# getreu/stringsext

Measured on AMD Instinct MI355X. Metric: GiB/s scanned, higher is better.
Workload: dtype u8

## Files before the change

stringsext_amd/csrc/sx_ctx.hpp:

```cpp
#pragma once
#include <hip/hip_runtime_api.h>
#include <stdio.h>
#include <stdlib.h>
#include <string.h>
#include <errno.h>
#include <fcntl.h>
#include <sys/mman.h>
#include <sys/stat.h>
#include <unistd.h>

#include <algorithm>
#include <atomic>
#include <chrono>
#include <condition_variable>
#include <deque>
#include <functional>
#include <mutex>
#include <string>
#include <thread>
#include <unordered_map>
#include <vector>

#include "sx_host.hpp"
#include "sx_switches.hpp"
// ... 81 lines not shown
    uint64_t* h_tot = nullptr;
    const uint32_t* grid_of_scan = nullptr; uint32_t grid_sub = 0; const uint8_t* grid_data = nullptr; uint64_t grid_len = 0;
    uint8_t* h_small = nullptr;
    std::vector<hipEvent_t> wave_ev;
};


}

struct sx_result {
    sx::Result r;
};

struct sx_ctx {
    std::shared_ptr<sx::PinnedPool> pool = std::make_shared<sx::PinnedPool>();
    std::shared_ptr<std::atomic<uint64_t>> dev_epoch = std::make_shared<std::atomic<uint64_t>>(0);
    std::vector<sx::Mission> missions;
    std::vector<sx::ScannerState> states;
    std::vector<sx::MissionDev> dev;
    bool host_only = false;
    bool sharded_call = false, single_piece = true;
    int device = -1;
    sx_options opt{};
    sx::Switches sw;
    std::string err;
    sx_stats stats{};
    hipStream_t scan_stream = nullptr, post_stream = nullptr;
    uint8_t* d_cache = nullptr;
    uint64_t d_cache_cap = 0;
    hipStream_t merge_copy_stream = nullptr;
    hipEvent_t merge_ev[3] = { nullptr, nullptr, nullptr };
    uint8_t* d_merge = nullptr; uint64_t d_merge_cap = 0, merge_out_room = 0, merge_n_out = 0;
    uint8_t* d_result = nullptr; uint64_t d_result_cap = 0;
    uint8_t* d_result_up = nullptr; uint64_t d_result_up_cap = 0;
    bool merge_async = false;
    bool merge_copy_pending[2] = { false, false };
    uint64_t merge_parts = 0;
    uint64_t merged_out_bytes = 0;
    double out_density = 0;
    hipEvent_t ev_interleaved = nullptr;
    std::atomic<bool> interleave_pending{ false };
    std::mutex mu;
    std::mutex err_mu;
    std::recursive_mutex grow_mu;
    void set_err(std::string text) { std::lock_guard<std::mutex> g(err_mu); err = std::move(text); }
    unsigned n_cus = 256, scan_blocks_per_cu = 8;
    hipStream_t copy_stream = nullptr;
    hipStream_t d2h_stream = nullptr;
    uint8_t* ing_pin[2] = { nullptr, nullptr };
    uint8_t* ing_dev[2] = { nullptr, nullptr };
    uint64_t ing_cap = 0, ing_dev_cap = 0;
    uint32_t region_cap = 64;
    std::vector<uint32_t> dense;
    uint8_t* d_input = nullptr;
    uint64_t d_input_cap = 0;
    uint64_t ondemand_fetches = 0;
    std::vector<uint64_t> last_runs;
    std::vector<char> wave_pred;
    std::vector<double> wave_density;
    std::vector<char> wave_off;
    std::vector<sx::RunList> shard_runs;
    bool shard_runs_valid = false;
    uint64_t shard_runs_off = 0, shard_runs_len = 0;
    const void* shard_runs_ptr = nullptr;
    uint8_t* h_pin = nullptr;   uint64_t h_pin_cap = 0;
    uint8_t* h_pin2 = nullptr;  uint64_t h_pin2_cap = 0;
    uint8_t* d_scratch = nullptr; uint64_t d_scratch_cap = 0;
};

#define HIP_TRY(ctx, expr)                                                                     \
    do {                                                                                       \
        hipError_t e_ = (expr);                                                                \
        if (e_ != hipSuccess) {                                                                \
            (ctx)->set_err(std::string(#expr) + ": " + hipGetErrorString(e_));                 \
            return SX_E_HIP;                                                                   \
        }                                                                                      \
    } while (0)

namespace sx {

class SparseDeviceBytes : public ByteView {
public:
    SparseDeviceBytes(sx_ctx* ctx, const uint8_t* d_base, uint64_t len = 0) : ctx_(ctx), d_base_(d_base), len_(len) {}
    void add(uint64_t lo, uint64_t hi, const uint8_t* p) { segs_.push_back({ lo, hi, p }); }
    void add_copy(uint64_t lo, uint64_t hi, const uint8_t* p) {
        owned_.emplace_back(p, p + (hi - lo));
        segs_.push_back({ lo, hi, owned_.back().data() });
    }
    bool empty() const { return segs_.empty(); }
    const uint8_t* span(uint64_t off, size_t n, size_t* hint) override {
        size_t a = *hint < segs_.size() ? *hint : 0;
        if (!(a < segs_.size() && segs_[a].lo <= off)) a = 0;
        size_t steps = 0;
        while (a < segs_.size() && segs_[a].hi <= off && steps < 8) { a++; steps++; }
        if (!(a < segs_.size() && segs_[a].lo <= off && off < segs_[a].hi)) {
            size_t lo = 0, hi = segs_.size();
            while (lo < hi) {
                size_t mid = (lo + hi) / 2;
                if (segs_[mid].hi <= off) lo = mid + 1; else hi = mid;
            }
            a = lo;
        }
        if (a < segs_.size() && segs_[a].lo <= off && off + n <= segs_[a].hi) { *hint = a; return segs_[a].p + (off - segs_[a].lo); }
        std::lock_guard<std::mutex> g(mu_);
        if (len_) {
            const uint64_t b = off / kBlock;
            if (off + n <= std::min<uint64_t>(len_, (b + 1) * kBlock)) {
                auto it = blocks_.find(b);
                if (it == blocks_.end()) {
                    const uint64_t lo = b * kBlock, hi = std::min<uint64_t>(len_, lo + kBlock);
                    std::vector<uint8_t> v((size_t)(hi - lo));
                    if (hipMemcpy(v.data(), d_base_ + lo, (size_t)(hi - lo), hipMemcpyDeviceToHost) != hipSuccess) memset(v.data(), 0, v.size());
                    ctx_->ondemand_fetches++;
                    it = blocks_.emplace(b, std::move(v)).first;
                }
                return it->second.data() + (off - b * kBlock);
            }
        }
        extra_.emplace_back(n);
        if (hipMemcpy(extra_.back().data(), d_base_ + off, n, hipMemcpyDeviceToHost) != hipSuccess)
            memset(extra_.back().data(), 0, n);
        ctx_->ondemand_fetches++;
        return extra_.back().data();
    }

private:
    struct Seg { uint64_t lo, hi; const uint8_t* p; };
    sx_ctx* ctx_;
    const uint8_t* d_base_;
    uint64_t len_ = 0;
    static constexpr uint64_t kBlock = 65536;
    std::unordered_map<uint64_t, std::vector<uint8_t>> blocks_;
    std::vector<Seg> segs_;
    std::deque<std::vector<uint8_t>> extra_, owned_;
    std::mutex mu_;
};

int ensure_pinned(sx_ctx* ctx, uint64_t bytes);
int ensure_pinned2(sx_ctx* ctx, uint64_t bytes);
int read_back_sync(sx_ctx* ctx, sx::MissionDev& d, hipStream_t s, void* host_dst, const void* dev_src, size_t bytes);
int read_back_async(sx_ctx* ctx, hipStream_t s, void* pinned_dst, const void* dev_src, size_t bytes);
int ensure_scratch(sx_ctx* ctx, uint64_t bytes);
int ensure_capacity(sx_ctx* ctx, ScanSlot& s, uint32_t cap);
int ensure_rp(sx_ctx* ctx, MissionDev& d, int slot, uint64_t bytes);
int ensure_cache(sx_ctx* ctx, uint64_t bytes);
unsigned usable_cpus();
unsigned replay_threads(const sx_ctx* ctx);
void begin_call(sx_ctx* ctx);

ScanParams scan_params(const sx_ctx* ctx, int mission, const ScanSlot& s, const uint8_t* d_bytes, uint64_t len,
                       uint32_t parity, uint64_t min_chars);
int stage_a_launch(sx_ctx* ctx, const std::vector<int>& which, const uint8_t* d_bytes, uint64_t len,
                   const std::vector<uint32_t>& parity, const std::vector<uint64_t>& min_chars, int si);
struct ReplayJob;
int ensure_copy_stream(sx_ctx* ctx);
bool result_stays_on_device(const sx_ctx* ctx, const ReplayJob& job);
int merge_drain(sx_ctx* ctx);
int stage_a_finish(sx_ctx* ctx, const std::vector<int>& which, const uint8_t* d_bytes, uint64_t len,
                   const std::vector<uint32_t>& parity, const std::vector<uint64_t>& min_chars, int si,
                   std::vector<RunList>* out, bool cut_into_pieces = false, const ReplayJob* wave_job = nullptr);
int device_runs(sx_ctx* ctx, const std::vector<int>& which, const uint8_t* d_bytes, uint64_t len,
                const std::vector<uint32_t>& parity, const std::vector<uint64_t>& min_chars,
                std::vector<RunList>* out);

struct ReplayJob {
    uint64_t len = 0;
    int file_id = -1;
    bool is_last = false;
    std::vector<uint64_t> lo;
    uint64_t hi = 0;
    std::vector<char> entry_exact;
    std::vector<uint64_t> consumed0, stream0;
    bool commit_state = true;
    uint32_t slice_base = 0;
    const uint8_t* d_bytes = nullptr;
};




struct PreReplayed {
    std::vector<char> done;
    std::vector<MissionFindings> per;
    std::vector<uint64_t> ends;
    explicit PreReplayed(size_t nm) : done(nm, 0), per(nm), ends(nm, 0) {}
};


constexpr int SX_WAVE_FALLBACK = 1001;
constexpr int SX_NEED_RUNS = 1002;
bool wave_replay_wanted(const sx_ctx* ctx, const ReplayJob& job, size_t k, size_t n_runs, uint64_t heavy_tiles = 0);
int wave_replay_mission(sx_ctx* ctx, size_t k, ByteView& view, const ReplayJob& job, MissionFindings* out, uint64_t* end_pos,
                        uint64_t defer_min_bytes, bool own_stream = false);
bool device_replay_wanted(const sx_ctx* ctx, const ReplayJob& job, size_t k, size_t n_runs);
int device_replay_mission(sx_ctx* ctx, size_t k, ByteView& view, const ReplayJob& job, const RunList& runs,
                          MissionFindings* out, uint64_t* end_pos, uint64_t defer_min_bytes);
int replay_all(sx_ctx* ctx, ByteView& bytes, const ReplayJob& job, const std::vector<RunList>& runs,
               Result* into, uint64_t* end_pos, PreReplayed* pre = nullptr);
ReplayJob whole_chunk_job(sx_ctx* ctx, uint64_t len, int file_id, bool is_last);
int download_for_replay(sx_ctx* ctx, const uint8_t* d_bytes, uint64_t len,
                        const std::vector<RunList>* runs_opt, SparseDeviceBytes* view,
                        const ReplayJob& job, const std::vector<char>* skip = nullptr,
                        bool* used_base = nullptr);

struct ResultHolder {
    sx_result* r = new sx_result();
    ~ResultHolder() { delete r; }
    sx_result* release() { sx_result* x = r; r = nullptr; return x; }
};

int set_entry_params(sx_ctx* ctx, bool carried_state_is_entry, const uint8_t* host_bytes, const uint8_t* d_bytes, uint64_t len,
                     uint64_t stream_off, std::vector<uint32_t>* parity);
int scan_common(sx_ctx* ctx, const uint8_t* host_bytes, const uint8_t* d_bytes, uint64_t len, int file_id,
                int is_last, sx_result** out, uint32_t slice_base0 = 0, sx_result* append_to = nullptr);
int shard_common(sx_ctx* ctx, const uint8_t* host_bytes, const uint8_t* d_bytes,
                 const sx_run* const* given_runs, const uint64_t* given_n, uint64_t buf_off, uint64_t buf_len,
                 uint64_t own_lo, uint64_t own_hi, const uint64_t* start_at, uint64_t file_stream_off, int file_id,
                 int reuse_runs, sx_result** out, uint64_t* end_pos);
int stream_core(sx_ctx* ctx, sx_read_fn read, void* read_user, uint64_t chunk_bytes, int input_file_id,
                sx_result_fn sink, void* sink_user, sx_result* accumulate, int is_last_at_eof,
                const uint8_t* direct = nullptr, uint64_t direct_len = 0);

}
```

stringsext_amd/csrc/sx_schedule.cpp:

```cpp
#include "sx_ctx.hpp"
#include <thread>

using namespace sx;

namespace sx {

uint64_t piece_bytes(const sx_ctx* ctx, uint64_t len) {
    uint64_t piece = 0;
    bool halves = false;
    if (ctx->sw.piece_mib >= 0) piece = (uint64_t)ctx->sw.piece_mib << 20;
    else if (len >= (16ull << 30) && ctx->missions.size() >= 2 && !(ctx->opt.flags & (SX_OPT_NO_FUSED_SCAN | SX_OPT_MISSION_STREAMS | SX_OPT_RESULT_ON_DEVICE))) {
        piece = ((len / 100) * 50 + kInputBufLen - 1) / kInputBufLen * kInputBufLen;
        halves = true;
    }
    if (piece == 0 || (!halves && len < 2 * piece)) return len;
    for (const Mission& m : ctx->missions) if (m.is_dbcs()) return len;
    return piece / kInputBufLen * kInputBufLen;
}

static uint64_t seq_piece_bytes(const sx_ctx* ctx, uint64_t len) {
    uint64_t piece = 0;
    if (ctx->sw.seq_piece_kib >= 0) {
        piece = (uint64_t)ctx->sw.seq_piece_kib << 10;
        if (piece == 0) return len;
    } else if (ctx->sw.seq_piece_mib >= 0) {
        piece = (uint64_t)ctx->sw.seq_piece_mib << 20;
        if (piece == 0) return len;
    } else {
        if (ctx->opt.flags & SX_OPT_RESULT_ON_DEVICE) return len;
        if (ctx->missions.size() < 2 || ctx->out_density <= 0) return len;
        const double out = ctx->out_density * (double)len;
        if (out < 4.0 * (double)(1ull << 30)) return len;
        const uint64_t n = (uint64_t)(out / (2.25 * (double)(1ull << 30))) + 1;
        piece = std::max<uint64_t>((len + n - 1) / n, 1ull << 30);
    }
    piece = std::max<uint64_t>((piece + kInputBufLen - 1) / kInputBufLen, 2) * kInputBufLen;
    return len < 2 * piece ? len : piece;
}

static int entry_param(sx_ctx* ctx, size_t k, const Decoder* carried, const uint8_t* host_bytes, const uint8_t* d_bytes,
                       uint64_t len, uint64_t stream_off, uint32_t* out, uint32_t* out_replay = nullptr) {
    const Mission& m = ctx->missions[k];
    *out = (uint32_t)(stream_off & 1);
    if (out_replay) *out_replay = 0;
    if (!m.is_dbcs()) return SX_OK;
    *out = 0;
    if (!carried || carried->idle() || len == 0) return SX_OK;
    uint8_t first[8] = { 0, 0, 0, 0, 0, 0, 0, 0 };
    const uint64_t n = std::min<uint64_t>(8, len);
    if (host_bytes) memcpy(first, host_bytes, n);
    else HIP_TRY(ctx, hipMemcpy(first, d_bytes, n, hipMemcpyDeviceToHost));
    *out = carried->entry_skip_scan(first, n);
    if (out_replay) *out_replay = carried->entry_skip(first, n);
    if (ctx->sw.debug_entry) { const DDecoder& dd = const_cast<Decoder*>(carried)->raw(); fprintf(stderr, "[sx] entry mission %zu: dlead %02x gb2 %02x gb3 %02x rq_n %u first %02x %02x -> scan %u replay %u\n", k, dd.dlead, dd.gb2, dd.gb3, dd.rq_n, first[0], first[1], *out, out_replay ? *out_replay : 0u); }
    return SX_OK;
}
int set_entry_params(sx_ctx* ctx, bool carried_state_is_entry, const uint8_t* host_bytes, const uint8_t* d_bytes, uint64_t len,
                     uint64_t stream_off, std::vector<uint32_t>* parity) {
    parity->clear();
    for (size_t k = 0; k < ctx->missions.size(); k++) {
        uint32_t ep = 0, ep_replay = 0;
        int rc = entry_param(ctx, k, carried_state_is_entry ? &ctx->states[k].decoder : nullptr, host_bytes, d_bytes, len,
                             stream_off, &ep, &ep_replay);
        if (rc != SX_OK) return rc;
        parity->push_back(ep);
        ctx->missions[k].buf_entry_skip = ctx->missions[k].is_dbcs() ? ep_replay : 0u;
    }
    return SX_OK;
}

void mission_order(sx_ctx* ctx, std::vector<int>* out) {
    const size_t nm = ctx->missions.size();
    std::vector<int>& order = *out;
    order.resize(nm);
    for (size_t k = 0; k < nm; k++) order[k] = (int)k;
    if (ctx->last_runs.size() != nm) return;
    std::stable_sort(order.begin(), order.end(), [&](int x, int y) { return ctx->last_runs[(size_t)x] > ctx->last_runs[(size_t)y]; });
    const int mode = ctx->sw.busiest_last;
    if (mode) std::reverse(order.begin(), order.end());
    if (mode == 2 && nm >= 3) std::swap(order[nm - 1], order[nm - 2]);
}

int sync_streams_and_return(sx_ctx* ctx, int rc) {
    ctx->merge_async = false;
    (void)merge_drain(ctx);
    for (auto& d : ctx->dev) { (void)hipStreamSynchronize(d.stream); (void)hipStreamSynchronize(d.stream_b); }
    return rc;
}

struct BufferScan {
    const uint8_t* host_bytes = nullptr;
    const uint8_t* d_bytes = nullptr;
    uint64_t len = 0;
    std::vector<int> order;
    std::vector<uint32_t> parity;
    std::vector<uint64_t> minc;
    int slot = 0;
    std::unique_ptr<SparseDeviceBytes> base_view;
    bool whole = false;
    bool skip_scan(const sx_ctx* ctx, size_t k) const {
        return whole && len >= 2 * kInputBufLen && k < ctx->wave_pred.size() && ctx->wave_pred[k] && ctx->missions[k].wave_ok && !ctx->sw.wave_keep_scan
               && ctx->sw.wave_replay != 0;
    }
    bool none_scanned(const sx_ctx* ctx) const {
        if (not_scanned.size() != ctx->missions.size()) return false;
        for (char c : not_scanned) if (!c) return false;
        return true;
    }

    int fetch_base(sx_ctx* ctx) {
        base_view.reset();
        if (host_bytes) return SX_OK;
        base_view.reset(new SparseDeviceBytes(ctx, d_bytes, len));
        if (none_scanned(ctx)) return SX_OK;
        ReplayJob none;
        return download_for_replay(ctx, d_bytes, len, nullptr, base_view.get(), none);
    }
    std::vector<char> not_scanned;
    int launch(sx_ctx* ctx) {
        not_scanned.assign(ctx->missions.size(), 0);
        std::vector<int> ks; std::vector<uint32_t> par; std::vector<uint64_t> mc;
        for (int k : order) {
            if (ctx->missions[(size_t)k].host_sequential() || skip_scan(ctx, (size_t)k)) { not_scanned[(size_t)k] = 1; continue; }
            ks.push_back(k); par.push_back(parity[(size_t)k]); mc.push_back(minc[(size_t)k]);
        }
        return ks.empty() ? SX_OK : stage_a_launch(ctx, ks, d_bytes, len, par, mc, slot);
    }
    int finish_and_replay(sx_ctx* ctx, const ReplayJob& job, const std::function<int()>& after_last_finish,
                          std::vector<RunList>* runs, Result* into, uint64_t* ends) {
        const size_t nm = ctx->missions.size();
        runs->assign(nm, RunList{});
        HostBytes host_view(host_bytes ? host_bytes : (const uint8_t*)"");
        ByteView& early_view = host_bytes ? (ByteView&)host_view : (ByteView&)*base_view;
        PreReplayed pre(nm);
        if (ctx->last_runs.size() != nm) ctx->last_runs.assign(nm, 0);
        ctx->wave_off.assign(nm, 0);
        if (ctx->wave_pred.size() != nm) ctx->wave_pred.assign(nm, 0);
        std::vector<std::thread> wave_threads(nm);
        std::vector<int> wave_rc(nm, SX_OK);
        std::vector<char> threaded(nm, 0);
        struct Joiner {
            std::vector<std::thread>& t;
            ~Joiner() { for (auto& x : t) if (x.joinable()) x.join(); }
        } joiner{ wave_threads };
        const uint64_t defer_all = nm >= 2 ? (result_stays_on_device(ctx, job) ? 1 : ctx->sw.defer_min_bytes) : 0;
        if (nm >= 2 && ctx->sw.wave_threads) {
            if (ctx->wave_density.size() != nm) ctx->wave_density.assign(nm, 0.0);
            for (size_t k = 0; k < nm; k++) {
                const bool unscanned = k < not_scanned.size() && not_scanned[k];
                if (ctx->missions[k].host_sequential() || !unscanned || !wave_replay_wanted(ctx, job, k, len)) continue;
                threaded[k] = 1;
                ctx->stats.bytes_scanned += len;
                wave_threads[k] = std::thread([ctx, k, &early_view, &job, &pre, &wave_rc, defer_all]() {
                    (void)hipSetDevice(ctx->device);
                    wave_rc[k] = wave_replay_mission(ctx, k, early_view, job, &pre.per[k], &pre.ends[k], defer_all, true);
                });
            }
        }
        std::vector<size_t> order2;
        for (size_t oi = 0; oi < nm; oi++) if (!threaded[(size_t)order[oi]]) order2.push_back((size_t)order[oi]);
        for (size_t oi = 0; oi < nm; oi++) if (threaded[(size_t)order[oi]]) order2.push_back((size_t)order[oi]);
        for (size_t oi = 0; oi < nm; oi++) {
            const size_t k = order2[oi];
            std::vector<RunList> one;
            int rc = SX_OK;
            const bool unscanned = k < not_scanned.size() && not_scanned[k];
            bool replayed = false;
            if (threaded[k]) {
                wave_threads[k].join();
                rc = wave_rc[k];
                if (rc == SX_WAVE_FALLBACK) {
                    ctx->wave_off[k] = 1; ctx->wave_pred[k] = 0;
                    ctx->stats.bytes_scanned -= len;
                    rc = SX_OK;
                } else if (rc != SX_OK) return rc;
                else replayed = true;
            }
            if (replayed) {
                one.assign(1, RunList{});
                one[0].n = len / 16; one[0].skipped = true; one[0].complete = true;
            } else if (ctx->missions[k].host_sequential()) {
                one.assign(1, RunList{});
                one[0].complete = true;
            } else if (unscanned && wave_replay_wanted(ctx, job, k, len)) {
                one.assign(1, RunList{});
                one[0].n = len / 16; one[0].skipped = true; one[0].complete = true;
                ctx->stats.bytes_scanned += len;
            } else {
                if (unscanned) {
                    ctx->wave_pred[k] = 0;
                    rc = stage_a_launch(ctx, { (int)k }, d_bytes, len, { parity[k] }, { minc[k] }, slot);
                    if (rc != SX_OK) return rc;
                }
                rc = stage_a_finish(ctx, { (int)k }, d_bytes, len, { parity[k] }, { minc[k] }, slot, &one, true, &job);
            }
            if (rc != SX_OK) return rc;
            (*runs)[k] = std::move(one[0]);
            if (!(*runs)[k].own.empty()) (*runs)[k].use_own();
            ctx->last_runs[k] = (*runs)[k].size();
            const bool last_mission = oi + 1 == nm;
            bool next_queued = false;
            auto queue_next = [&]() -> int {
                if (!last_mission || !after_last_finish || next_queued) return SX_OK;
                next_queued = true;
                return after_last_finish();
            };
            if (!(*runs)[k].skipped && (rc = queue_next()) != SX_OK) return rc;
            if (replayed) { pre.done[k] = 1; if ((rc = queue_next()) != SX_OK) return rc; continue; }
            if (device_replay_wanted(ctx, job, k, (*runs)[k].size())) {
                SX_TL("mission %zu: device replay begins (%zu runs)", k, (*runs)[k].size());
                rc = device_replay_mission(ctx, k, early_view, job, (*runs)[k], &pre.per[k], &pre.ends[k], defer_all);
                SX_TL("mission %zu: device replay done", k);
                if (rc == SX_NEED_RUNS) {
                    ctx->wave_off[k] = 1;
                    rc = stage_a_launch(ctx, { (int)k }, d_bytes, len, { parity[k] }, { minc[k] }, slot);
                    if (rc == SX_OK) rc = stage_a_finish(ctx, { (int)k }, d_bytes, len, { parity[k] }, { minc[k] }, slot, &one, true, nullptr);
                    if (rc != SX_OK) return rc;
                    (*runs)[k] = std::move(one[0]);
                    if (!(*runs)[k].own.empty()) (*runs)[k].use_own();
                    ctx->last_runs[k] = (*runs)[k].size();
                    if ((rc = queue_next()) != SX_OK) return rc;
                    if (!device_replay_wanted(ctx, job, k, (*runs)[k].size())) continue;
                    rc = device_replay_mission(ctx, k, early_view, job, (*runs)[k], &pre.per[k], &pre.ends[k], defer_all);
                }
                if (rc != SX_OK) return rc;
                pre.done[k] = 1;
            }
            if ((rc = queue_next()) != SX_OK) return rc;
        }
        SX_TL("all missions finished / replayed on the device");
        if (host_bytes) return replay_all(ctx, host_view, job, *runs, into, ends, &pre);
        SparseDeviceBytes view(ctx, d_bytes, len);
        bool base_is_enough = false;
        int rc = download_for_replay(ctx, d_bytes, len, runs, &view, job, &pre.done, &base_is_enough);
        if (rc != SX_OK) return rc;
        return replay_all(ctx, base_is_enough ? (ByteView&)*base_view : (ByteView&)view, job, *runs, into, ends, &pre);
    }
};

int scan_common(sx_ctx* ctx, const uint8_t* host_bytes, const uint8_t* d_bytes, uint64_t len, int file_id,
                       int is_last, sx_result** out, uint32_t slice_base0, sx_result* append_to) {
    const double t_begin = now_ms();
    g_tl_on = ctx->sw.timeline; g_tl_t0 = t_begin;
    SX_TL("scan_common: %llu bytes", (unsigned long long)len);
    const size_t nm = ctx->missions.size();
    ctx->dev_epoch->fetch_add(1);
    ctx->shard_runs_valid = false;
    std::vector<uint64_t> stream0(nm);
    for (size_t k = 0; k < nm; k++) stream0[k] = ctx->states[k].stream_bytes;
    std::vector<int> order;
    mission_order(ctx, &order);
    const uint64_t seq_piece = ctx->host_only ? len : seq_piece_bytes(ctx, len);
    const bool seq = seq_piece < len;
    const uint64_t piece = seq ? seq_piece : piece_bytes(ctx, len);
    const uint64_t n_pieces = len ? (len + piece - 1) / piece : 1;
    ctx->single_piece = n_pieces == 1 && !append_to;
    const uint64_t merged0 = ctx->merged_out_bytes;
    int entry_rc = SX_OK;
    auto make = [&](uint64_t p) {
        BufferScan b;
        const uint64_t off = p * piece;
        b.host_bytes = host_bytes ? host_bytes + off : nullptr;
        b.d_bytes = d_bytes + off;
        b.len = std::min(piece, len - off);
        b.order = order;
        b.whole = true;
        b.slot = (int)(p & 1);
        for (size_t k = 0; k < nm; k++) {
            uint32_t ep = (uint32_t)((stream0[k] + off) & 1);
            if (ctx->missions[k].is_dbcs()) {
                uint32_t ep_replay = 0;
                entry_rc = std::min(entry_rc, entry_param(ctx, k, &ctx->states[k].decoder, b.host_bytes, b.d_bytes, b.len, 0, &ep, &ep_replay));
                ctx->missions[k].buf_entry_skip = ep_replay;
            }
            b.parity.push_back(ep);
            b.minc.push_back(ctx->missions[k].long_run);
        }
        return b;
    };
    ResultHolder res;
    int rc = SX_OK;
    if (seq) {
        ctx->merge_async = true;
        ctx->stats.seq_pieces += n_pieces;
        for (uint64_t p = 0; p < n_pieces; p++) {
            BufferScan b = make(p);
            if (entry_rc != SX_OK) return sync_streams_and_return(ctx, entry_rc);
            if ((rc = b.launch(ctx)) != SX_OK) return sync_streams_and_return(ctx, rc);
            if ((rc = b.fetch_base(ctx)) != SX_OK) return sync_streams_and_return(ctx, rc);
            ReplayJob job = whole_chunk_job(ctx, b.len, file_id, is_last != 0 && p + 1 == n_pieces);
            job.d_bytes = b.d_bytes;
            job.slice_base = slice_base0 + (uint32_t)(p * piece / kInputBufLen);
            std::vector<RunList> runs;
            rc = b.finish_and_replay(ctx, job, nullptr, &runs, append_to ? &append_to->r : &res.r->r, nullptr);
            if (rc != SX_OK) return sync_streams_and_return(ctx, rc);
        }
        ctx->merge_async = false;
        if ((rc = merge_drain(ctx)) != SX_OK) return sync_streams_and_return(ctx, rc);
        if (len) ctx->out_density = (double)(ctx->merged_out_bytes - merged0) / (double)len;
        ctx->stats.total_ms = now_ms() - t_begin;
        if (!append_to) *out = res.release();
        return SX_OK;
    }
    std::vector<BufferScan> pieces;
    for (uint64_t p = 0; p < n_pieces; p++) pieces.push_back(make(p));
    if (entry_rc != SX_OK) return entry_rc;
    uint64_t launched = 0;
    for (; launched < std::min<uint64_t>(2, n_pieces); launched++)
        if ((rc = pieces[launched].launch(ctx)) != SX_OK) return sync_streams_and_return(ctx, rc);
    SX_TL("scans queued");
    if ((rc = pieces[0].fetch_base(ctx)) != SX_OK) return sync_streams_and_return(ctx, rc);
    SX_TL("base fetched");
    for (uint64_t p = 0; p < n_pieces; p++) {
        BufferScan& b = pieces[p];
        if (p > 0 && (rc = b.fetch_base(ctx)) != SX_OK) return sync_streams_and_return(ctx, rc);
        ReplayJob job = whole_chunk_job(ctx, b.len, file_id, is_last != 0 && p + 1 == n_pieces);
        job.d_bytes = b.d_bytes;
        job.slice_base = slice_base0 + (uint32_t)(p * piece / kInputBufLen);
        std::vector<RunList> runs;
        rc = b.finish_and_replay(ctx, job,
                                 [&]() -> int { return launched < n_pieces ? pieces[launched++].launch(ctx) : SX_OK; },
                                 &runs, append_to ? &append_to->r : &res.r->r, nullptr);
        if (rc != SX_OK) return sync_streams_and_return(ctx, rc);
    }
    if (len) ctx->out_density = (double)(ctx->merged_out_bytes - merged0) / (double)len;
    ctx->stats.total_ms = now_ms() - t_begin;
    SX_TL("scan_common done");
    if (!append_to) *out = res.release();
    return SX_OK;
}


int shard_common(sx_ctx* ctx, const uint8_t* host_bytes, const uint8_t* d_bytes,
                        const sx_run* const* given_runs, const uint64_t* given_n, uint64_t buf_off, uint64_t buf_len,
                        uint64_t own_lo, uint64_t own_hi, const uint64_t* start_at, uint64_t file_stream_off, int file_id,
                        int reuse_runs, sx_result** out, uint64_t* end_pos) {
    if (!out || !end_pos || (buf_off % kInputBufLen) != 0 || own_lo < buf_off || own_hi < own_lo || own_hi > buf_off + buf_len) {
        ctx->err = "bad shard geometry"; return SX_E_INVALID;
    }
    ctx->sharded_call = true;
    const size_t nm = ctx->missions.size();
    const double t_begin = now_ms();
    for (const Mission& m : ctx->missions)
        if (m.host_sequential()) {
            ctx->err = "an ISO-2022-JP mission cannot be sharded: the character set in force at a shard start depends on every escape "
                       "sequence in front of it (its stage B is one sequential pass)";
            return SX_E_INVALID;
        }
    for (const Mission& m : ctx->missions)
        if (m.c.chars_min_nb == 0 && buf_off != 0) {
            ctx->err = "a mission with chars_min_nb 0 cannot be sharded: its state at a shard start cannot be derived from the bytes "
                       "in front of it (stage B runs as one sequential pass for it)";
            return SX_E_INVALID;
        }
    if (buf_off > 0) {
        bool any = false;
        for (const Mission& m : ctx->missions) any = any || m.is_dbcs();
        if (any) {
            const uint64_t front = own_lo - buf_off;
            std::vector<char> found(nm, 0);
            std::vector<uint8_t> tmp;
            auto all_found = [&]() { for (size_t k = 0; k < nm; k++) if (ctx->missions[k].is_dbcs() && !found[k]) return false; return true; };
            for (uint64_t at = 0; at < front && !all_found(); at += 65536) {
                const uint64_t n = std::min<uint64_t>(65536, front - at);
                const uint8_t* s = host_bytes ? host_bytes + at : nullptr;
                if (!s) {
                    tmp.resize(n);
                    HIP_TRY(ctx, hipMemcpy(tmp.data(), d_bytes + at, n, hipMemcpyDeviceToHost));
                    s = tmp.data();
                }
                for (size_t k = 0; k < nm; k++) {
                    const Mission& m = ctx->missions[k];
                    if (!m.is_dbcs() || found[k]) continue;
                    const int enc = m.c.encoding;
                    const bool two = enc_family((uint32_t)enc) == 4;
                    for (uint64_t i = 0; i < n; i++)
                        if (!(two ? dbcs_may_be_pending_after<4>(s[i], enc) : dbcs_may_be_pending_after<5>(s[i], enc))) { found[k] = 1; break; }
                }
            }
            if (!all_found()) {
                ctx->err = "no byte outside the lead range between the buffer start and own_lo: the token grid of a double-byte "
                           "mission is unknown there; repeat with a larger halo in front";
                return SX_E_HALO;
            }
        }
    }
    if (given_runs) {
        ctx->shard_runs.assign(nm, RunList{});
        for (size_t k = 0; k < nm; k++) ctx->shard_runs[k].assign(given_runs[k], given_runs[k] + given_n[k]);
    }
    const void* buf_id = d_bytes ? (const void*)d_bytes : (const void*)host_bytes;
    const bool same_buffer = ctx->shard_runs_valid && ctx->shard_runs_off == buf_off && ctx->shard_runs_len == buf_len && ctx->shard_runs_ptr == buf_id;
    const bool scan_now = !given_runs && !(reuse_runs && same_buffer);
    if (given_runs || scan_now) ctx->shard_runs_valid = false;
    BufferScan b;
    {
        int rc = set_entry_params(ctx, buf_off == 0, host_bytes, d_bytes, buf_len, file_stream_off + buf_off, &b.parity);
        if (rc != SX_OK) return rc;
    }
    if (scan_now) {
        b.host_bytes = host_bytes; b.d_bytes = d_bytes; b.len = buf_len; mission_order(ctx, &b.order); b.slot = 0;
        for (size_t k = 0; k < nm; k++) b.minc.push_back(ctx->missions[k].long_run);
        int rc = b.launch(ctx);
        if (rc == SX_OK) rc = b.fetch_base(ctx);
        if (rc != SX_OK) return sync_streams_and_return(ctx, rc);
    }

    ReplayJob job;
    job.len = buf_len; job.file_id = file_id; job.is_last = false;
    job.hi = own_hi - buf_off;
    job.commit_state = job.hi >= buf_len;
    job.slice_base = (uint32_t)(buf_off / kInputBufLen);
    for (size_t k = 0; k < nm; k++) {
        uint64_t lo = own_lo;
        if (start_at && start_at[k] > lo) lo = start_at[k];
        if (lo > own_hi) lo = own_hi;
        job.lo.push_back(lo - buf_off);
        job.entry_exact.push_back(buf_off == 0 && lo == 0);
        job.consumed0.push_back(ctx->missions[k].c.counter_offset + file_stream_off + buf_off);
        job.stream0.push_back(file_stream_off + buf_off);
    }
    job.d_bytes = d_bytes;
    int rc;
    ResultHolder res;
    std::vector<uint64_t> ends(nm, 0);
    if (scan_now) {
        ctx->shard_runs_valid = false;
        rc = b.finish_and_replay(ctx, job, nullptr, &ctx->shard_runs, &res.r->r, ends.data());
        if (rc != SX_OK) return sync_streams_and_return(ctx, rc);
        ctx->shard_runs_valid = true; ctx->shard_runs_off = buf_off; ctx->shard_runs_len = buf_len; ctx->shard_runs_ptr = buf_id;
    } else if (host_bytes) {
        HostBytes view(host_bytes);
        rc = replay_all(ctx, view, job, ctx->shard_runs, &res.r->r, ends.data());
    } else {
        SparseDeviceBytes view(ctx, d_bytes, buf_len);
        rc = download_for_replay(ctx, d_bytes, buf_len, &ctx->shard_runs, &view, job);
        if (rc != SX_OK) return rc;
        rc = replay_all(ctx, view, job, ctx->shard_runs, &res.r->r, ends.data());
    }
    if (rc == SX_OK) *out = res.release();
    for (size_t k = 0; k < nm; k++) end_pos[k] = buf_off + ends[k];
    ctx->stats.total_ms = now_ms() - t_begin;
    return rc;
}


}
```

stringsext_amd/csrc/sx_stage_a.cpp:

```cpp
#include "sx_ctx.hpp"

using namespace sx;

namespace sx {

static bool large_regions_fit(uint64_t len, uint64_t n_regions, uint32_t cap) {
    const uint64_t slots = n_regions * cap;
    return slots < (1ull << 31) && slots * sizeof(DevRun) <= std::max<uint64_t>(256ull << 20, len / 2);
}

static uint32_t subchunk_bytes(const sx_ctx* ctx) {
    const uint32_t sub = ctx->opt.subchunk_bytes ? ctx->opt.subchunk_bytes : 256u * 1024u;
    return std::max<uint32_t>(kTileBytes, sub / kTileBytes * kTileBytes);
}

static bool fusion_allowed(const sx_ctx* ctx) {
    return !(ctx->opt.flags & (SX_OPT_NO_FUSED_SCAN | SX_OPT_MISSION_STREAMS)) && !ctx->sw.mission_streams && ctx->sw.fused && ctx->sw.scan_warm < 0;
}

ScanParams scan_params(const sx_ctx* ctx, int mission, const ScanSlot& s, const uint8_t* d_bytes, uint64_t len,
                       uint32_t parity, uint64_t min_chars) {
    const Mission& m = ctx->missions[(size_t)mission];
    ScanParams p = m.proto;
    p.data = d_bytes; p.len = len; p.subchunk = subchunk_bytes(ctx); p.parity = parity;
    p.pair_lut = ctx->dev[(size_t)mission].d_pair_lut;
    if (p.gb4) {
        p.gb_ranges = ctx->dev[(size_t)mission].d_table ? ctx->dev[(size_t)mission].d_table + kGbN : nullptr;
        p.ubf = m.c.ubf;
        if (!p.gb_ranges) p.gb4 = 0;
    }
    p.wave_prio = ctx->sw.scan_prio;
    p.min_chars = (uint32_t)std::min<uint64_t>(min_chars, kRecCharsMask);
    if (p.min_chars == 0) p.min_chars = 1;
    p.cand_bytes = std::min<uint32_t>(p.min_chars * (m.is_utf16() ? 2u : 1u), 14u);
    {
        uint32_t have = 1;
        for (int i = 0; i < 5; i++) {
            const uint32_t sh = have < p.cand_bytes ? std::min(have, p.cand_bytes - have) : 0;
            p.cand_sh[i] = sh;
            have += sh;
        }
    }
    p.capacity = s.capacity; p.recs = s.d_recs; p.counters = s.d_counters;
    p.region_cap = s.region_cap; p.region_counts = s.d_cnt; p.grid_flags = s.d_grid;
    unsigned occ = ctx->scan_blocks_per_cu;
    p.persistent = (occ >= 1 && occ < 8) ? occ * ctx->n_cus : 0u;
    return p;
}

int stage_a_launch(sx_ctx* ctx, const std::vector<int>& which, const uint8_t* d_bytes, uint64_t len,
                   const std::vector<uint32_t>& parity, const std::vector<uint64_t>& min_chars, int si) {
    if (len == 0) return SX_OK;
    for (size_t k = 0; k < which.size(); k++) {
        MissionDev& d = ctx->dev[(size_t)which[k]];
        ScanSlot& s = d.slot[si];
        if (s.free_pending) { HIP_TRY(ctx, hipStreamWaitEvent(d.stream, s.ev_free, 0)); s.free_pending = false; }
        {
            const uint32_t sub = subchunk_bytes(ctx);
            const uint64_t n_regions = (len + sub - 1) / sub;
            if (ctx->dense.size() != ctx->missions.size()) ctx->dense.assign(ctx->missions.size(), 0);
            s.region_cap = 0; s.n_regions = n_regions;
            const uint32_t dn = ctx->dense[(size_t)which[k]];
            const uint32_t want_cap = dn > 1 ? dn : (dn == 0 ? ctx->region_cap : 0u);
            if (ctx->region_cap && want_cap &&
                (dn > 1 ? large_regions_fit(len, n_regions, want_cap) : n_regions * want_cap < (1ull << 28))) {
                s.region_cap = want_cap;
                int rc = ensure_capacity(ctx, s, (uint32_t)(n_regions * s.region_cap));
                if (rc != SX_OK && dn > 1) {
                    (void)hipGetLastError();
                    ctx->dense[(size_t)which[k]] = 1;
                    s.region_cap = 0;
                    rc = SX_OK;
                }
                if (rc != SX_OK) return rc;
                if (s.region_cap == 0) goto launch;
                if (s.cnt_cap < n_regions) {
                    if (s.d_cnt) HIP_TRY(ctx, hipFree(s.d_cnt));
                    s.d_cnt = nullptr; s.cnt_cap = 0;
                    HIP_TRY(ctx, hipMalloc((void**)&s.d_cnt, (n_regions + n_regions / 4 + 64) * 4));
                    s.cnt_cap = n_regions + n_regions / 4 + 64;
                }
            }
        }
    launch:
        const bool dbcs = ctx->missions[(size_t)which[k]].is_dbcs();
        if (dbcs) {
            const uint32_t sub = subchunk_bytes(ctx);
            const uint64_t n_sub = (len + sub - 1) / sub;
            if (s.grid_cap < n_sub) {
                if (s.d_grid) HIP_TRY(ctx, hipFree(s.d_grid));
                s.d_grid = nullptr; s.grid_cap = 0;
                HIP_TRY(ctx, hipMalloc((void**)&s.d_grid, (n_sub + n_sub / 4 + 64) * 4));
                s.grid_cap = n_sub + n_sub / 4 + 64;
            }
        }
    }
    std::vector<char> fused(which.size(), 0);
    std::vector<ScanParams> params(which.size());
    for (size_t k = 0; k < which.size(); k++)
        params[k] = scan_params(ctx, which[k], ctx->dev[(size_t)which[k]].slot[si], d_bytes, len, parity[k], min_chars[k]);
    if (fusion_allowed(ctx)) {
        FusedParams fp{};
        uint32_t used = 0;
        size_t member[kFusedMax] = { 0, 0, 0 };
        for (size_t k = 0; k < which.size(); k++) {
            if (params[k].persistent) continue;
            const int sl = fused_slot_of(ctx->missions[(size_t)which[k]].kind, params[k]);
            if (sl < 0 || (used >> sl) & 1u) continue;
            if (sl >= 1 && (used & 6u) && ((fp.m[(used & 2u) ? 1 : 2].parity ^ params[k].parity) & 1u)) continue;
            used |= 1u << sl; fp.m[sl] = params[k]; member[sl] = k;
        }
        if (__builtin_popcount(used) >= 2 || used == 1u) {
            hipStream_t st = nullptr;
            for (int sl = 0; sl < kFusedMax; sl++) if ((used >> sl) & 1u) {
                MissionDev& d = ctx->dev[(size_t)which[member[sl]]];
                if (!st) st = d.stream;
                HIP_TRY(ctx, hipMemsetAsync(d.slot[si].d_counters, 0, kCounterWords * sizeof(uint32_t), st));
            }
            for (int sl = 0; sl < kFusedMax; sl++) if ((used >> sl) & 1u) HIP_TRY(ctx, hipEventRecord(ctx->dev[(size_t)which[member[sl]]].slot[si].ev0, st));
            HIP_TRY(ctx, launch_scan_fused(fp, used, st, ctx->sw.fused_prefilter));
            bool first = true;
            for (int sl = 0; sl < kFusedMax; sl++) if ((used >> sl) & 1u) {
                ScanSlot& s = ctx->dev[(size_t)which[member[sl]]].slot[si];
                HIP_TRY(ctx, hipEventRecord(s.ev1, st));
                s.fused = true; s.fused_first = first; first = false;
                fused[member[sl]] = 1;
            }
            ctx->stats.fused_launches++;
        }
    }
    for (size_t k = 0; k < which.size(); k++) {
        if (fused[k]) continue;
        MissionDev& d = ctx->dev[(size_t)which[k]];
        ScanSlot& s = d.slot[si];
        s.fused = false; s.fused_first = false;
        const bool dbcs = ctx->missions[(size_t)which[k]].is_dbcs();
        const ScanParams& p = params[k];
        const uint64_t n_sub = (len + p.subchunk - 1) / p.subchunk;
        for (int w = ctx->sw.scan_warm; w > 0; w--) {
            if (dbcs) HIP_TRY(ctx, hipMemsetAsync(s.d_grid, 0, n_sub * 4, d.stream));
            HIP_TRY(ctx, hipMemsetAsync(s.d_counters, 0, kCounterWords * sizeof(uint32_t), d.stream));
            HIP_TRY(ctx, launch_scan(ctx->missions[(size_t)which[k]].kind, p, d.stream));
        }
        if (dbcs) HIP_TRY(ctx, hipMemsetAsync(s.d_grid, 0, n_sub * 4, d.stream));
        HIP_TRY(ctx, hipMemsetAsync(s.d_counters, 0, kCounterWords * sizeof(uint32_t), d.stream));
        HIP_TRY(ctx, hipEventRecord(s.ev0, d.stream));
        HIP_TRY(ctx, launch_scan(ctx->missions[(size_t)which[k]].kind, p, d.stream));
        HIP_TRY(ctx, hipEventRecord(s.ev1, d.stream));
        if (dbcs) { d.grid_of_scan = s.d_grid; d.grid_sub = p.subchunk; d.grid_data = d_bytes; d.grid_len = len; }
    }
    return SX_OK;
}

int stage_a_finish(sx_ctx* ctx, const std::vector<int>& which, const uint8_t* d_bytes, uint64_t len,
                   const std::vector<uint32_t>& parity, const std::vector<uint64_t>& min_chars, int si,
                   std::vector<RunList>* out, bool cut_into_pieces, const ReplayJob* wave_job) {
    out->assign(which.size(), RunList{});
    if (len == 0) return SX_OK;
    const double t0 = now_ms();
    for (size_t k = 0; k < which.size(); k++) {
        MissionDev& d = ctx->dev[(size_t)which[k]];
        ScanSlot& s = d.slot[si];
        HIP_TRY(ctx, hipEventSynchronize(s.ev1));
        const double t_ev = now_ms();
        SX_TL("mission %d: scan kernel done", which[k]);
        float ms = 0;
        HIP_TRY(ctx, hipEventElapsedTime(&ms, s.ev0, s.ev1));
        if (which[k] < 16) ctx->stats.kernel_ms[which[k]] += ms;
        if (s.fused && s.fused_first) ctx->stats.fused_ms += ms;
        if (which[k] < 64) { if (s.fused) ctx->stats.fused_mask |= 1ull << which[k]; else ctx->stats.fused_mask &= ~(1ull << which[k]); }
// ... 180 lines not shown
```

stringsext_amd/csrc/sx_switches.cpp:

```cpp
#include "sx_switches.hpp"

#include <stdio.h>
#include <stdlib.h>

#include <algorithm>

namespace sx {

static bool present(const char* name) { return getenv(name) != nullptr; }
static bool on_unless_0(const char* name) { const char* e = getenv(name); return !(e && !atoi(e)); }
static bool on_if_nonzero(const char* name) { const char* e = getenv(name); return e && atoi(e); }
static int int_or(const char* name, int unset) { const char* e = getenv(name); return e ? atoi(e) : unset; }
static int64_t i64_or(const char* name, int64_t unset) { const char* e = getenv(name); return e ? (int64_t)atoll(e) : unset; }
static int clamped_or(const char* name, int lo, int hi, int unset) { const char* e = getenv(name); return e ? std::max(lo, std::min(hi, atoi(e))) : unset; }
static uint64_t u64_at_least(const char* name, uint64_t lo, uint64_t unset) { const char* e = getenv(name); return e ? std::max<uint64_t>(lo, (uint64_t)atoll(e)) : unset; }

Switches Switches::from_env() {
    Switches s;
    if (const char* e = getenv("SX_PIN_FLAGS")) s.pin_flags = (int64_t)(unsigned)strtoul(e, nullptr, 0);
    s.small_copy = on_unless_0("SX_SMALL_COPY");
    if (const char* e = getenv("SX_REPLAY_THREADS")) s.replay_threads = (int)std::max(1u, std::min(256u, (unsigned)atoi(e)));
    s.result_on_device = on_if_nonzero("SX_RESULT_ON_DEVICE");
    s.scan_blocks_per_cu = int_or("SX_SCAN_BLOCKS_PER_CU", s.scan_blocks_per_cu);
    if (const char* e = getenv("SX_REGION_CAP")) s.region_cap = (int64_t)(uint32_t)atoi(e);
    s.scan_cus = clamped_or("SX_SCAN_CUS", 1, INT32_MAX, s.scan_cus);
    if (const char* e = getenv("SX_PRIO")) s.prio_n = std::max(0, sscanf(e, "%d,%d", &s.prio_scan, &s.prio_post));
    s.mission_streams = present("SX_MISSION_STREAMS");
    s.scan_prio = (uint32_t)int_or("SX_SCAN_PRIO", (int)s.scan_prio);
    s.fused = on_unless_0("SX_FUSED");
    s.fused_prefilter = int_or("SX_FUSED_PREFILTER", s.fused_prefilter);
    s.scan_warm = clamped_or("SX_SCAN_WARM", 0, INT32_MAX, s.scan_warm);
    s.no_large_regions = present("SX_NO_LARGE_REGIONS");
    s.device_join_min = (uint32_t)int_or("SX_DEVICE_JOIN_MIN", (int)s.device_join_min);
    s.no_pieces = present("SX_NO_PIECES");
    s.probe_rot = (uint32_t)int_or("SX_PROBE_ROT", (int)s.probe_rot);
    s.host_replay = present("SX_HOST_REPLAY");
    s.device_replay = present("SX_DEVICE_REPLAY");
    s.host_stitch = present("SX_HOST_STITCH");
    s.no_replay_skip = present("SX_NO_REPLAY_SKIP");
    s.no_grid_bound = present("SX_NO_GRID_BOUND");
    s.no_replay_cache = present("SX_NO_REPLAY_CACHE");
    s.max_region_windows = (uint32_t)clamped_or("SX_MAX_REGION_WINDOWS", 1, INT32_MAX, (int)s.max_region_windows);
    s.replay_cache_mib = i64_or("SX_REPLAY_CACHE_MIB", s.replay_cache_mib);
    s.fast_replay = on_unless_0("SX_FAST_REPLAY");
    s.count_waves = int_or("SX_COUNT_WAVES", s.count_waves);
    s.stitch_block = clamped_or("SX_STITCH_BLOCK", 0, INT32_MAX, s.stitch_block);
    s.slabs = clamped_or("SX_SLABS", 1, 64, s.slabs);
    s.replay_copy_wgs = int_or("SX_REPLAY_COPY_WGS", s.replay_copy_wgs);
    s.host_merge = present("SX_HOST_MERGE");
    s.packed = on_unless_0("SX_PACKED");
    s.merge_part_mib = u64_at_least("SX_MERGE_PART_MIB", 1, s.merge_part_mib);
    s.merge_part_findings = u64_at_least("SX_MERGE_PART_FINDINGS", 1024, s.merge_part_findings);
    s.merge_copy_wgs = int_or("SX_MERGE_COPY_WGS", s.merge_copy_wgs);
    s.merge_copy_nt = int_or("SX_MERGE_COPY_NT", s.merge_copy_nt);
    s.merge_copy_threads = clamped_or("SX_MERGE_COPY_THREADS", 64, 1024, s.merge_copy_threads);
    s.host_merge_seg_bytes = u64_at_least("SX_HOST_MERGE_SEG_BYTES", 1, s.host_merge_seg_bytes);
    s.splice_seg_bytes = u64_at_least("SX_SPLICE_SEG_BYTES", 1, s.splice_seg_bytes);
    s.piece_mib = i64_or("SX_PIECE_MIB", s.piece_mib);
    s.seq_piece_kib = i64_or("SX_SEQ_PIECE_KIB", s.seq_piece_kib);
    s.seq_piece_mib = i64_or("SX_SEQ_PIECE_MIB", s.seq_piece_mib);
    s.debug_entry = present("SX_DEBUG_ENTRY");
    s.busiest_last = int_or("SX_BUSIEST_LAST", s.busiest_last);
    if (const char* e = getenv("SX_DEFER_MIN_BYTES")) s.defer_min_bytes = (uint64_t)atoll(e);
    s.wave_threads = on_unless_0("SX_WAVE_THREADS");
    s.timeline = int_or("SX_TIMELINE", s.timeline);
    s.timing = present("SX_TIMING");
    s.timing2 = present("SX_TIMING2");
    if (const char* e = getenv("SX_WAVE_REPLAY")) s.wave_replay = atoi(e) != 0;
    s.wave_keep_scan = present("SX_WAVE_KEEP_SCAN");
    if (const char* e = getenv("SX_WAVE_BYTES_PER_RUN")) s.wave_bytes_per_run = (uint64_t)atoll(e);
    s.wave_stream_prio = int_or("SX_WAVE_STREAM_PRIO", s.wave_stream_prio);
    s.wave_batches = clamped_or("SX_WAVE_BATCHES", 1, 64, s.wave_batches);
    s.wave_slabs = clamped_or("SX_WAVE_SLABS", 1, 64, s.wave_slabs);
    s.wave_lut = on_if_nonzero("SX_WAVE_LUT");
    s.wave_desc = on_unless_0("SX_WAVE_DESC");
    s.wave_desc_cap = clamped_or("SX_WAVE_DESC_CAP", 1, INT32_MAX, s.wave_desc_cap);
    s.wave_fail = present("SX_WAVE_FAIL");
    if (const char* e = getenv("SX_WAVE_REPAIR")) s.wave_repair = atoi(e) ? std::max(1, atoi(e)) : 0;
    s.wave_same = on_unless_0("SX_WAVE_SAME");
    if (const char* e = getenv("SX_SCAN_STREAM_MIB")) s.scan_stream_mib = (uint64_t)atoll(e);
    s.ingest_mmap = present("SX_INGEST_MMAP");
    return s;
}

}
```

stringsext_amd/csrc/sx_switches.hpp:

```cpp
#pragma once
#include <stdint.h>

namespace sx {

struct Switches {
    int64_t pin_flags = -1;
    bool small_copy = true;
    int replay_threads = 0;
    bool result_on_device = false;
    int scan_blocks_per_cu = -1;
    int64_t region_cap = -1;
    int scan_cus = 0;
    int prio_n = -1, prio_scan = 0, prio_post = 0;
    bool mission_streams = false;
    uint32_t scan_prio = 0;
    bool fused = true;
    int fused_prefilter = -1;
    int scan_warm = -1;
    bool no_large_regions = false;
    uint32_t device_join_min = 65536;
    bool no_pieces = false;
    uint32_t probe_rot = 0;
    bool host_replay = false;
    bool device_replay = false;
    bool host_stitch = false;
    bool no_replay_skip = false;
    bool no_grid_bound = false;
    bool no_replay_cache = false;
    uint32_t max_region_windows = 0;
    int64_t replay_cache_mib = -1;
    bool fast_replay = true;
    int count_waves = 4;
    int stitch_block = 0;
    int slabs = 0;
    int replay_copy_wgs = 0;
    bool host_merge = false;
    bool packed = true;
    uint64_t merge_part_mib = 0;
    uint64_t merge_part_findings = 0;
    int merge_copy_wgs = -1;
    int merge_copy_nt = 1;
    int merge_copy_threads = 512;
    uint64_t host_merge_seg_bytes = 0;
    uint64_t splice_seg_bytes = 0;
    int64_t piece_mib = -1;
    int64_t seq_piece_kib = -1;
    int64_t seq_piece_mib = -1;
    bool debug_entry = false;
    int busiest_last = 0;
    uint64_t defer_min_bytes = 256ull << 20;
    bool wave_threads = true;
    int timeline = 0;
    bool timing = false;
    bool timing2 = false;
    int wave_replay = -1;
    bool wave_keep_scan = false;
    uint64_t wave_bytes_per_run = 0;
    int wave_stream_prio = -1;
    int wave_batches = 0;
    int wave_slabs = 0;
    bool wave_lut = false;
    bool wave_desc = true;
    int wave_desc_cap = 0;
    bool wave_fail = false;
    int wave_repair = -1;
    bool wave_same = true;
    uint64_t scan_stream_mib = 0;
    bool ingest_mmap = false;

    static Switches from_env();
};

}
```

Baseline: 4000.

## Plan scan pieces by share list and batch stage-A finish across fused missions

Replaces the fixed-size piece computation with a piece_plan that cuts the input at boundaries given by share weights (env SX_PIECE_PLAN) or by fixed MiB, defaulting to halves for large fused scans. The fused default now depends on whether a fused launch is actually expected. When all missions use the fused slot, stage A is finished for all of them in one call and the next piece is queued right after, instead of waiting on each mission in turn. This aims to overlap the next piece's scan with replay sooner, at the cost of more complex scheduling and new per-piece offset bookkeeping.

```diff
diff --git a/stringsext_amd/csrc/sx_ctx.hpp b/stringsext_amd/csrc/sx_ctx.hpp
--- a/stringsext_amd/csrc/sx_ctx.hpp
+++ b/stringsext_amd/csrc/sx_ctx.hpp
@@ -257,6 +257,7 @@
                        uint32_t parity, uint64_t min_chars);
 int stage_a_launch(sx_ctx* ctx, const std::vector<int>& which, const uint8_t* d_bytes, uint64_t len,
                    const std::vector<uint32_t>& parity, const std::vector<uint64_t>& min_chars, int si);
+bool fused_launch_expected(const sx_ctx* ctx);
 struct ReplayJob;
 int ensure_copy_stream(sx_ctx* ctx);
 bool result_stays_on_device(const sx_ctx* ctx, const ReplayJob& job);
@@ -314,6 +315,7 @@
     sx_result* release() { sx_result* x = r; r = nullptr; return x; }
 };
 
+void piece_plan(uint64_t len, const uint32_t* shares, size_t n_shares, int64_t piece_mib, bool fused, bool dbcs, std::vector<uint64_t>* ends);
 int set_entry_params(sx_ctx* ctx, bool carried_state_is_entry, const uint8_t* host_bytes, const uint8_t* d_bytes, uint64_t len,
                      uint64_t stream_off, std::vector<uint32_t>* parity);
 int scan_common(sx_ctx* ctx, const uint8_t* host_bytes, const uint8_t* d_bytes, uint64_t len, int file_id,
diff --git a/stringsext_amd/csrc/sx_schedule.cpp b/stringsext_amd/csrc/sx_schedule.cpp
--- a/stringsext_amd/csrc/sx_schedule.cpp
+++ b/stringsext_amd/csrc/sx_schedule.cpp
@@ -5,17 +5,34 @@
 
 namespace sx {
 
-uint64_t piece_bytes(const sx_ctx* ctx, uint64_t len) {
-    uint64_t piece = 0;
-    bool halves = false;
-    if (ctx->sw.piece_mib >= 0) piece = (uint64_t)ctx->sw.piece_mib << 20;
-    else if (len >= (16ull << 30) && ctx->missions.size() >= 2 && !(ctx->opt.flags & (SX_OPT_NO_FUSED_SCAN | SX_OPT_MISSION_STREAMS | SX_OPT_RESULT_ON_DEVICE))) {
-        piece = ((len / 100) * 50 + kInputBufLen - 1) / kInputBufLen * kInputBufLen;
-        halves = true;
-    }
-    if (piece == 0 || (!halves && len < 2 * piece)) return len;
-    for (const Mission& m : ctx->missions) if (m.is_dbcs()) return len;
-    return piece / kInputBufLen * kInputBufLen;
+static const uint32_t kDefaultShares[] = { 1, 1 };
+void piece_plan(uint64_t len, const uint32_t* shares, size_t n_shares, int64_t piece_mib, bool fused, bool dbcs, std::vector<uint64_t>* ends) {
+    ends->clear();
+    auto by_shares = [&](const uint32_t* sh, size_t n) {
+        uint64_t sum = 0, cum = 0;
+        for (size_t i = 0; i < n; i++) sum += sh[i];
+        for (size_t i = 0; i + 1 < n && sum; i++) {
+            cum += sh[i];
+            const uint64_t at = ((len / sum) * cum + (len % sum) * cum / sum + kInputBufLen - 1) / kInputBufLen * kInputBufLen;
+            if (at < len && at > (ends->empty() ? 0 : ends->back())) ends->push_back(at);
+        }
+    };
+    if (dbcs || len == 0) { }
+    else if (n_shares) by_shares(shares, n_shares);
+    else if (piece_mib >= 0) {
+        const uint64_t piece = ((uint64_t)piece_mib << 20) / kInputBufLen * kInputBufLen;
+        if (piece && len >= 2 * ((uint64_t)piece_mib << 20)) for (uint64_t at = piece; at < len; at += piece) ends->push_back(at);
+    } else if (fused && len >= (16ull << 30)) by_shares(kDefaultShares, sizeof kDefaultShares / sizeof kDefaultShares[0]);
+    ends->push_back(len);
+}
+
+std::vector<uint64_t> piece_ends(const sx_ctx* ctx, uint64_t len) {
+    bool dbcs = false;
+    for (const Mission& m : ctx->missions) dbcs = dbcs || m.is_dbcs();
+    const bool fused = !(ctx->opt.flags & SX_OPT_RESULT_ON_DEVICE) && fused_launch_expected(ctx);
+    std::vector<uint64_t> ends;
+    piece_plan(len, ctx->sw.piece_plan, (size_t)ctx->sw.piece_plan_n, ctx->sw.piece_mib, fused, dbcs, &ends);
+    return ends;
 }
 
 static uint64_t seq_piece_bytes(const sx_ctx* ctx, uint64_t len) {
@@ -160,6 +177,32 @@
         std::vector<size_t> order2;
         for (size_t oi = 0; oi < nm; oi++) if (!threaded[(size_t)order[oi]]) order2.push_back((size_t)order[oi]);
         for (size_t oi = 0; oi < nm; oi++) if (threaded[(size_t)order[oi]]) order2.push_back((size_t)order[oi]);
+        bool next_queued = false;
+        auto queue_now = [&]() -> int {
+            if (!after_last_finish || next_queued) return SX_OK;
+            next_queued = true;
+            return after_last_finish();
+        };
+        bool batch = nm >= 2 && len > 0;
+        for (size_t k = 0; k < nm && batch; k++)
+            batch = !threaded[k] && !ctx->missions[k].host_sequential() && !(k < not_scanned.size() && not_scanned[k]) && ctx->dev[k].slot[slot].fused;
+        if (batch) {
+            std::vector<int> ks; std::vector<uint32_t> par; std::vector<uint64_t> mc;
+            for (size_t k : order2) { ks.push_back((int)k); par.push_back(parity[k]); mc.push_back(minc[k]); }
+            std::vector<RunList> all;
+            int rc = stage_a_finish(ctx, ks, d_bytes, len, par, mc, slot, &all, true, &job);
+            if (rc != SX_OK) return rc;
+            bool counted_only = false;
+            for (size_t oi = 0; oi < nm; oi++) {
+                const size_t k = order2[oi];
+                (*runs)[k] = std::move(all[oi]);
+                if (!(*runs)[k].own.empty()) (*runs)[k].use_own();
+                ctx->last_runs[k] = (*runs)[k].size();
+                counted_only = counted_only || (*runs)[k].skipped;
+            }
+            if (!counted_only && (rc = queue_now()) != SX_OK) return rc;
+            SX_TL("stage A finished for all missions%s", next_queued ? ", next piece queued" : "");
+        }
         for (size_t oi = 0; oi < nm; oi++) {
             const size_t k = order2[oi];
             std::vector<RunList> one;
@@ -176,7 +219,8 @@
                 } else if (rc != SX_OK) return rc;
                 else replayed = true;
             }
-            if (replayed) {
+            if (batch) {
+            } else if (replayed) {
                 one.assign(1, RunList{});
                 one[0].n = len / 16; one[0].skipped = true; one[0].complete = true;
             } else if (ctx->missions[k].host_sequential()) {
@@ -195,16 +239,13 @@
                 rc = stage_a_finish(ctx, { (int)k }, d_bytes, len, { parity[k] }, { minc[k] }, slot, &one, true, &job);
             }
             if (rc != SX_OK) return rc;
-            (*runs)[k] = std::move(one[0]);
-            if (!(*runs)[k].own.empty()) (*runs)[k].use_own();
-            ctx->last_runs[k] = (*runs)[k].size();
+            if (!batch) {
+                (*runs)[k] = std::move(one[0]);
+                if (!(*runs)[k].own.empty()) (*runs)[k].use_own();
+                ctx->last_runs[k] = (*runs)[k].size();
+            }
             const bool last_mission = oi + 1 == nm;
-            bool next_queued = false;
-            auto queue_next = [&]() -> int {
-                if (!last_mission || !after_last_finish || next_queued) return SX_OK;
-                next_queued = true;
-                return after_last_finish();
-            };
+            auto queue_next = [&]() -> int { return last_mission ? queue_now() : SX_OK; };
             if (!(*runs)[k].skipped && (rc = queue_next()) != SX_OK) return rc;
             if (replayed) { pre.done[k] = 1; if ((rc = queue_next()) != SX_OK) return rc; continue; }
             if (device_replay_wanted(ctx, job, k, (*runs)[k].size())) {
@@ -252,17 +293,19 @@
     mission_order(ctx, &order);
     const uint64_t seq_piece = ctx->host_only ? len : seq_piece_bytes(ctx, len);
     const bool seq = seq_piece < len;
-    const uint64_t piece = seq ? seq_piece : piece_bytes(ctx, len);
-    const uint64_t n_pieces = len ? (len + piece - 1) / piece : 1;
+    std::vector<uint64_t> ends;
+    if (seq) { for (uint64_t at = seq_piece; at < len; at += seq_piece) ends.push_back(at); ends.push_back(len); }
+    else ends = piece_ends(ctx, len);
+    const uint64_t n_pieces = ends.size();
     ctx->single_piece = n_pieces == 1 && !append_to;
     const uint64_t merged0 = ctx->merged_out_bytes;
     int entry_rc = SX_OK;
     auto make = [&](uint64_t p) {
         BufferScan b;
-        const uint64_t off = p * piece;
+        const uint64_t off = p ? ends[p - 1] : 0;
         b.host_bytes = host_bytes ? host_bytes + off : nullptr;
         b.d_bytes = d_bytes + off;
-        b.len = std::min(piece, len - off);
+        b.len = ends[p] - off;
         b.order = order;
         b.whole = true;
         b.slot = (int)(p & 1);
@@ -290,7 +333,7 @@
             if ((rc = b.fetch_base(ctx)) != SX_OK) return sync_streams_and_return(ctx, rc);
             ReplayJob job = whole_chunk_job(ctx, b.len, file_id, is_last != 0 && p + 1 == n_pieces);
             job.d_bytes = b.d_bytes;
-            job.slice_base = slice_base0 + (uint32_t)(p * piece / kInputBufLen);
+            job.slice_base = slice_base0 + (uint32_t)((p ? ends[p - 1] : 0) / kInputBufLen);
             std::vector<RunList> runs;
             rc = b.finish_and_replay(ctx, job, nullptr, &runs, append_to ? &append_to->r : &res.r->r, nullptr);
             if (rc != SX_OK) return sync_streams_and_return(ctx, rc);
@@ -316,7 +359,7 @@
         if (p > 0 && (rc = b.fetch_base(ctx)) != SX_OK) return sync_streams_and_return(ctx, rc);
         ReplayJob job = whole_chunk_job(ctx, b.len, file_id, is_last != 0 && p + 1 == n_pieces);
         job.d_bytes = b.d_bytes;
-        job.slice_base = slice_base0 + (uint32_t)(p * piece / kInputBufLen);
+        job.slice_base = slice_base0 + (uint32_t)((p ? ends[p - 1] : 0) / kInputBufLen);
         std::vector<RunList> runs;
         rc = b.finish_and_replay(ctx, job,
                                  [&]() -> int { return launched < n_pieces ? pieces[launched++].launch(ctx) : SX_OK; },
@@ -446,3 +489,10 @@
 
 
 }
+
+extern "C" int sxt_piece_plan(uint64_t len, const uint32_t* shares, int n_shares, int64_t piece_mib, int fused, int dbcs, uint64_t* out, int cap) {
+    std::vector<uint64_t> ends;
+    sx::piece_plan(len, shares, n_shares > 0 ? (size_t)n_shares : 0, piece_mib, fused != 0, dbcs != 0, &ends);
+    for (size_t i = 0; i < ends.size() && (int)i < cap; i++) out[i] = ends[i];
+    return (int)ends.size();
+}
diff --git a/stringsext_amd/csrc/sx_stage_a.cpp b/stringsext_amd/csrc/sx_stage_a.cpp
--- a/stringsext_amd/csrc/sx_stage_a.cpp
+++ b/stringsext_amd/csrc/sx_stage_a.cpp
@@ -16,6 +16,20 @@
 
 static bool fusion_allowed(const sx_ctx* ctx) {
     return !(ctx->opt.flags & (SX_OPT_NO_FUSED_SCAN | SX_OPT_MISSION_STREAMS)) && !ctx->sw.mission_streams && ctx->sw.fused && ctx->sw.scan_warm < 0;
+}
+
+bool fused_launch_expected(const sx_ctx* ctx) {
+    if (!fusion_allowed(ctx) || ctx->region_cap == 0 || (ctx->scan_blocks_per_cu >= 1 && ctx->scan_blocks_per_cu < 8)) return false;
+    uint32_t used = 0;
+    for (size_t k = 0; k < ctx->missions.size(); k++) {
+        const Mission& m = ctx->missions[k];
+        if (m.host_sequential() || (ctx->dense.size() == ctx->missions.size() && ctx->dense[k] == 1)) continue;
+        ScanParams p = m.proto;
+        p.region_cap = ctx->region_cap; p.persistent = 0;
+        const int sl = fused_slot_of(m.kind, p);
+        if (sl >= 0) used |= 1u << sl;
+    }
+    return __builtin_popcount(used) >= 2;
 }
 
 ScanParams scan_params(const sx_ctx* ctx, int mission, const ScanSlot& s, const uint8_t* d_bytes, uint64_t len,
diff --git a/stringsext_amd/csrc/sx_switches.cpp b/stringsext_amd/csrc/sx_switches.cpp
--- a/stringsext_amd/csrc/sx_switches.cpp
+++ b/stringsext_amd/csrc/sx_switches.cpp
@@ -57,6 +57,17 @@
     s.host_merge_seg_bytes = u64_at_least("SX_HOST_MERGE_SEG_BYTES", 1, s.host_merge_seg_bytes);
     s.splice_seg_bytes = u64_at_least("SX_SPLICE_SEG_BYTES", 1, s.splice_seg_bytes);
     s.piece_mib = i64_or("SX_PIECE_MIB", s.piece_mib);
+    if (const char* e = getenv("SX_PIECE_PLAN")) {
+        for (const char* q = e; *q && s.piece_plan_n < 16;) {
+            char* end = nullptr;
+            const long v = strtol(q, &end, 10);
+            if (end == q || v < 1 || v > 65535) { s.piece_plan_n = 0; break; }
+            s.piece_plan[s.piece_plan_n++] = (uint32_t)v;
+            if (*end != ',') { if (*end) s.piece_plan_n = 0; break; }
+            q = end + 1;
+        }
+        if (s.piece_plan_n < 2) s.piece_plan_n = 0;
+    }
     s.seq_piece_kib = i64_or("SX_SEQ_PIECE_KIB", s.seq_piece_kib);
     s.seq_piece_mib = i64_or("SX_SEQ_PIECE_MIB", s.seq_piece_mib);
     s.debug_entry = present("SX_DEBUG_ENTRY");
diff --git a/stringsext_amd/csrc/sx_switches.hpp b/stringsext_amd/csrc/sx_switches.hpp
--- a/stringsext_amd/csrc/sx_switches.hpp
+++ b/stringsext_amd/csrc/sx_switches.hpp
@@ -44,6 +44,7 @@
     uint64_t host_merge_seg_bytes = 0;
     uint64_t splice_seg_bytes = 0;
     int64_t piece_mib = -1;
+    uint32_t piece_plan[16] = { 0 }; int piece_plan_n = 0;
     int64_t seq_piece_kib = -1;
     int64_t seq_piece_mib = -1;
     bool debug_entry = false;
```

Result: no change. 3998 (-0.0%).
